# tomas-gr/RawNanoporeSignalCompression

Hardware: AMD Instinct MI355X
Metric: MSamples/s encode+decode (1/2/4/8 GPU) at fixed ratio; % HBM roofline (higher is better)
Workload: dtype int16; 1 GPU; configs[1]: 100000 reads x 100000 int16 samples per GPU (1 chunk each), C5 encode+decode; reads_per_gpu=100000, samples_per_read=100000, global_reads=100000, parallelism=dp1 (reads round-robin, no data-path collective)

## Files before the change

rawnanoporesignalcompression_amd/csrc/pgn_kernels.hip:

```cpp
#include <hip/hip_runtime.h>
#include <stdio.h>
#include <stdlib.h>
#include <string.h>

#include <algorithm>
#include <condition_variable>
#include <mutex>
#include <vector>

#include "../../include/pgnano_hip.h"
#include "../../include/pgnano_pod5.h"
#include "pgn_c5.h"
#include "pgn_internal.h"
#include "pgn_select.h"
#include "pgn_vbz.h"
#include "pgn_variants.h"
#include "pgn_zdec.h"
#include "pgn_zenc.h"

namespace pgn {

constexpr uint32_t kPassSamples = 262144;
static_assert(PGN_MAX_CHUNK_SAMPLES >= kPassSamples, "chunk limits");
constexpr uint32_t kMaxEncSeq = (uint32_t)z1::kMaxSrc / 4 + 2;
// ... 2140 lines not shown
    case kCodecC4: hipLaunchKernelGGL(enc_chunk_kernel<kCodecC4>, dim3((unsigned)slots), dim3(64), 0, s, a); break;
    case kCodecC1: hipLaunchKernelGGL(enc_chunk_kernel<kCodecC1>, dim3((unsigned)slots), dim3(64), 0, s, a); break;
    case kCodecC2: hipLaunchKernelGGL(enc_chunk_kernel<kCodecC2>, dim3((unsigned)slots), dim3(64), 0, s, a); break;
    case kCodecC3: hipLaunchKernelGGL(enc_chunk_kernel<kCodecC3>, dim3((unsigned)slots), dim3(64), 0, s, a); break;
    case kCodecVbz0: hipLaunchKernelGGL(enc_chunk_kernel<kCodecVbz0>, dim3((unsigned)slots), dim3(64), 0, s, a); break;
    default: return PGN_ERR_INVALID_ARG;
    }
    HIPCHK(hipGetLastError());
    return PGN_OK;
}

static int launch_decode_fused(pgn_ctx* c, int codec, size_t nchunks, const uint8_t* d_in, const uint64_t* d_in_offsets,
                               const uint64_t* d_in_sizes, const DecOut& d_samples, const uint64_t* d_sample_offsets,
                               const uint32_t* d_sample_counts, int32_t* d_status, hipStream_t s)
{
    const size_t slots = nchunks < c->decFusedSlotsMax ? nchunks : c->decFusedSlotsMax;
    int rc = ensure_dec(c, slots, 0);
    if (rc) return rc;
    HIPCHK(hipEventRecord(c->ev[2], s));
    rc = ensure_queues(c, 1, s);
    if (rc) return rc;
    DecArgs a{};
    a.nchunks = nchunks;
    a.in = d_in;
    a.inOffsets = d_in_offsets;
    a.inSizes = d_in_sizes;
    set_out(a, d_samples);
    a.sampleOffsets = d_sample_offsets;
    a.sampleCounts = d_sample_counts;
    a.status = d_status;
    a.slotScratch = c->decScratch;
    a.slotBytes = dec_slot_bytes();
    a.prof = c->prof ? c->prof + kPhases : nullptr;
    a.queue = c->qCur;
    a.capN = kPassSamples;
    a.list = nullptr;
    c->lastUnits = nullptr;
    return launch_dec_chunks(codec, a, slots, s);
}

static int launch_dec_chunks(int codec, const DecArgs& a, size_t slots, hipStream_t s)
{
    switch (codec) {
    case kCodecC5: hipLaunchKernelGGL(dec_chunk_kernel<kCodecC5>, dim3((unsigned)slots), dim3(64), 0, s, a); break;
    case kCodecVbz: hipLaunchKernelGGL(dec_chunk_kernel<kCodecVbz>, dim3((unsigned)slots), dim3(64), 0, s, a); break;
    case kCodecC4: hipLaunchKernelGGL(dec_chunk_kernel<kCodecC4>, dim3((unsigned)slots), dim3(64), 0, s, a); break;
    case kCodecC1: hipLaunchKernelGGL(dec_chunk_kernel<kCodecC1>, dim3((unsigned)slots), dim3(64), 0, s, a); break;
    case kCodecC2: hipLaunchKernelGGL(dec_chunk_kernel<kCodecC2>, dim3((unsigned)slots), dim3(64), 0, s, a); break;
    case kCodecC3: hipLaunchKernelGGL(dec_chunk_kernel<kCodecC3>, dim3((unsigned)slots), dim3(64), 0, s, a); break;
    case kCodecVbz0: hipLaunchKernelGGL(dec_chunk_kernel<kCodecVbz0>, dim3((unsigned)slots), dim3(64), 0, s, a); break;
    default: return PGN_ERR_INVALID_ARG;
    }
    HIPCHK(hipGetLastError());
    return PGN_OK;
}

static int launch_encode_impl(pgn_ctx* c, int codec, size_t nchunks, const int16_t* d_samples, const uint64_t* d_sample_offsets,
                         const uint32_t* d_sample_counts, uint8_t* d_out, const uint64_t* d_out_offsets,
                         const uint64_t* d_out_caps, uint64_t* d_out_sizes, int32_t* d_status, uint64_t* d_stats,
                         void* stream)
{
    HIPCHK(hipSetDevice(c->device));
    hipStream_t s = stream ? (hipStream_t)stream : c->stream;
    const bool staged = c->encStaged || (!c->encForced && nchunks <= c->encStagedBelow);
    if (!staged || (codec != kCodecC5 && codec != kCodecVbz))
        return launch_encode_fused(c, codec, nchunks, d_samples, d_sample_offsets, d_sample_counts, d_out, d_out_offsets,
                                   d_out_caps, d_out_sizes, d_status, d_stats, s);
    const size_t G = nchunks < c->subBatch ? nchunks : c->subBatch;
    const size_t passes = (nchunks + G - 1) / G;
    const uint32_t nu = codec == kCodecVbz ? 1u : (uint32_t)kStreams;
    const size_t slots = nu * G < c->encSlotsMax ? nu * G : c->encSlotsMax;
    const size_t nbuf = passes > 1 ? 2 : 1;
    int rc = ensure_enc(c, slots, nbuf * G);
    if (rc) return rc;
    HIPCHK(hipEventRecord(c->ev[0], s));
    rc = ensure_queues(c, passes, s);
    if (rc) return rc;
    const hipStream_t sideS = passes > 1 ? c->side : s;
    if (passes > 1) {
        HIPCHK(hipEventRecord(c->evFork, s));
        HIPCHK(hipStreamWaitEvent(c->side, c->evFork, 0));
    }
    const size_t bufBytes = G * (kChunkStreamBytes + kChunkFrameBytes + 2 * 4 * kStreams);
    EncArgs a;
    a.nchunks = nchunks;
    a.samples = d_samples;
    a.sampleOffsets = d_sample_offsets;
    a.sampleCounts = d_sample_counts;
    a.out = d_out;
    a.outOffsets = d_out_offsets;
    a.outCaps = d_out_caps;
    a.outSizes = d_out_sizes;
    a.status = d_status;
    a.stats = d_stats;
    a.slotScratch = c->encScratch;
    a.slotBytes = enc_slot_bytes();
    a.epochs = c->epochs;
    a.prof = c->prof;
    a.G = G;
    a.nu = nu;
    a.capN = kPassSamples;
    a.list = nullptr;
    a.lookback = nullptr;
    a.epoch = 0;
    if (passes == 1 && G <= kSplitWgMaxChunks && codec != kCodecVbz) {
        rc = take_lookback(c, s, a.lookback, a.epoch);
        if (rc) return rc;
    }
    for (size_t p = 0; p < passes; p++) {
        const int b = (int)(p & 1);
        uint8_t* buf = c->encChunks + (size_t)b * bufBytes;
        a.streams = buf;
        a.frames = buf + G * kChunkStreamBytes;
        a.sizes = (uint32_t*)(a.frames + G * kChunkFrameBytes);
        a.fsizes = a.sizes + G * kStreams;
        a.base = p * G;
        a.queue = c->qCur + p;
        if (p >= 2) HIPCHK(hipStreamWaitEvent(c->side, c->evFree[b], 0));
        if (codec == kCodecVbz) hipLaunchKernelGGL(vbz_split_kernel, dim3((unsigned)G), dim3(64), 0, sideS, a);
        else if (a.lookback)
            hipLaunchKernelGGL(enc_split_lb_kernel, dim3((unsigned)(G * kSplitRanges)), dim3(64), 0, sideS, a);
        else hipLaunchKernelGGL(enc_split_kernel, dim3((unsigned)G), dim3(64), 0, sideS, a);
        if (passes > 1) {
            HIPCHK(hipEventRecord(c->evStage[b], c->side));
            HIPCHK(hipStreamWaitEvent(s, c->evStage[b], 0));
        }
        const bool coop = G <= kSplitWgMaxChunks && (size_t)nu * G <= slots;
        if (coop)
            hipLaunchKernelGGL(enc_zstd_coop_kernel, dim3((unsigned)(nu * G)), dim3(64 * kCoopEncWaves), 0, s, a);
        else hipLaunchKernelGGL(enc_zstd_kernel, dim3((unsigned)slots), dim3(64), 0, s, a);
        if (codec == kCodecVbz) hipLaunchKernelGGL(vbz_assemble_kernel, dim3((unsigned)G), dim3(64), 0, s, a);
        else if (!(coop && a.lookback)) hipLaunchKernelGGL(enc_assemble_kernel, dim3((unsigned)G), dim3(64), 0, s, a);
        if (passes > 1) HIPCHK(hipEventRecord(c->evFree[b], s));
    }
    HIPCHK(hipGetLastError());
    return PGN_OK;
}

#define PGN_LAUNCH_MERGE_PA(T)                                                                                           \
    do {                                                                                                                 \
        if (codec == kCodecVbz) hipLaunchKernelGGL(vbz_merge_pa_kernel<T>, dim3((unsigned)G), dim3(64), 0, ms, a);       \
        else if (a.lookback)                                                                                             \
            hipLaunchKernelGGL(dec_merge_lb_pa_kernel<T>, dim3((unsigned)(G * kMergeRanges)), dim3(64), 0, ms, a);       \
        else hipLaunchKernelGGL(dec_merge_pa_kernel<T>, dim3((unsigned)G), dim3(64), 0, ms, a);                          \
    } while (0)
static void launch_merge(int codec, const DecArgs& a, size_t G, hipStream_t ms)
{
    if (a.outType == PGN_OUT_F32) PGN_LAUNCH_MERGE_PA(float);
    else if (a.outType == PGN_OUT_F16) PGN_LAUNCH_MERGE_PA(_Float16);
    else if (codec == kCodecVbz) hipLaunchKernelGGL(vbz_merge_kernel, dim3((unsigned)G), dim3(64), 0, ms, a);
    else if (a.lookback)
        hipLaunchKernelGGL(dec_merge_lb_kernel, dim3((unsigned)(G * kMergeRanges)), dim3(64), 0, ms, a);
    else hipLaunchKernelGGL(dec_merge_kernel, dim3((unsigned)G), dim3(64), 0, ms, a);
}

static int launch_decode_impl(pgn_ctx* c, int codec, size_t nchunks, const uint8_t* d_in, const uint64_t* d_in_offsets,
                         const uint64_t* d_in_sizes, const DecOut& d_samples, const uint64_t* d_sample_offsets,
                         const uint32_t* d_sample_counts, int32_t* d_status, void* stream, uint32_t capCall)
{
    HIPCHK(hipSetDevice(c->device));
    hipStream_t s = stream ? (hipStream_t)stream : c->stream;
    if (!c->decStaged || (codec != kCodecC5 && codec != kCodecVbz))
        return launch_decode_fused(c, codec, nchunks, d_in, d_in_offsets, d_in_sizes, d_samples, d_sample_offsets,
                                   d_sample_counts, d_status, s);
    bool defer = codec == kCodecC5 && nchunks >= c->deferMin;
    const size_t stride = chunk_inter_bytes(capCall);
    size_t G = nchunks < c->subBatch ? nchunks : c->subBatch;
// ... 1186 lines not shown
```

rawnanoporesignalcompression_amd/csrc/pgn_zenc.h:

```cpp
#pragma once
#ifndef PGN_AB_SKIP
#define PGN_AB_SKIP 0
#endif
#include "pgn_c5.h"
#include "pgn_wave.h"
#include "zstd1_model.h"

namespace pgn {

constexpr int kWinWords = 392;
constexpr int kFiltSlots = 512;

struct WCTable {
    uint32_t tableLog;
    uint16_t stateTable[64];
    uint32_t deltaNbBits[16];
    int32_t deltaFindState[16];
};

struct alignas(16) EncLds {
    union {
        struct {
            uint64_t filt[kFiltSlots];
            uint32_t vh0[64], vh1[64], vpk[64];
            uint32_t vd0[64], vd1[64];
        };
        struct {
            uint32_t hist2[2][256];
            union {
            uint32_t hist2x[1 + 2 * 256];
            struct {
            uint8_t nbBits[256];
            uint16_t val[256];
            union {
                struct {
                    z1::HufNode nodes[2 * 256 + 4];
                    union {
                        uint32_t count[256];
                        struct {
                            uint16_t tanc[256];
                            uint16_t tdep[256];
                        };
                    };
                    uint32_t rankLast[16];
                    uint32_t vpr[16];
                };
                struct {
                    uint8_t weights[256];
                    uint8_t hdr[256];
                    WCTable fct;
                    uint8_t fscratch[64];
                    uint32_t wcount[16];
                    int16_t wnorm[16];
                    uint32_t wcumul[16];
                };
                struct {
                    uint32_t win[kWinWords];
                    uint32_t cw[256];
                };
            };
            };
            };
        };
        struct {
            z1::FseCTable sct[3];
            uint8_t stsym[512];
            uint32_t scount[3][64];
            int16_t snorm[64];
            uint32_t scumul[64];
            uint8_t snc[128];
            uint32_t sv[3][64];
            uint8_t sc[3][64];
        };
    };
    uint32_t u[8];
};
__device__ __forceinline__ uint32_t seg_count(const EncLds& L, int k, int s)
{
    return (L.hist2[k >> 1][s] >> (16 * (k & 1))) & 0xFFFFu;
}

static_assert(sizeof(EncLds) <= kCodecLdsBytes, "encoder LDS exceeds the codec LDS");
static_assert(__builtin_offsetof(EncLds, hdr) % 4 == 0, "table description words");
#define sEnc (*reinterpret_cast<EncLds*>(sCodecLds))

struct EncScratch {
    uint32_t* ht;
    z1::Seq* seqs;
    uint8_t* codes;
    uint8_t* lit;
    uint8_t* seqSection;
    z1::SeqWork* seqWork;
    uint32_t maxSeq;
    uint32_t* huf;
    struct CoopEncCmd __attribute__((address_space(3)))* coop;
};

__device__ inline uint32_t wave_match_count(const uint8_t* src, uint32_t a, uint32_t b, uint32_t end)
{
    const uint32_t o = 4u * (uint32_t)lane_id();
    uint32_t n = 0;
    while (a + n < end) {
        const uint32_t len = end - (a + n);
        const uint32_t nv = len > o ? (len - o < 4u ? len - o : 4u) : 0u;
        const int32_t so = (int32_t)len - 4 < (int32_t)o ? (int32_t)len - 4 : (int32_t)o;
        const uint32_t wa = ld32u(src + (int64_t)(a + n) + so), wb = ld32u(src + (int64_t)(b + n) + so);
        const uint32_t sh = 8u * (uint32_t)((int32_t)o - so);
        uint32_t x = nv ? ((wa ^ wb) >> sh) : 0u;
        x &= nv >= 4u ? 0xFFFFFFFFu : ((1u << (8u * nv)) - 1u);
        const uint32_t mism = x ? o + ((uint32_t)__builtin_ctz(x) >> 3) : 0xFFFFFFFFu;
        const uint64_t mm = ballot(mism != 0xFFFFFFFFu);
        if (mm) return n + readlane_u32(mism, __builtin_ctzll(mm));
        if (len <= 256u) return len + n;
        n += 256;
    }
    return n;
}

constexpr uint32_t kTagShift = 27;
constexpr uint32_t kTagEpochs = 1u << (32 - kTagShift);
constexpr uint32_t kMaxIdxBits = 26;
constexpr size_t kMaxFrameBytes = ((size_t)1 << kMaxIdxBits) - 2;
__host__ __device__ inline uint32_t ht_idx_bits(uint32_t frameN)
{
    if (frameN + 2 < (1u << 17)) return 17u;
    if (frameN + 2 < (1u << 20)) return 20u;
    uint32_t b = 21;
    while (b < kMaxIdxBits && frameN + 2 >= (1u << b)) b++;
    return b;
}
__device__ inline uint32_t ht_fp(uint32_t bytes, uint32_t idxBits)
{
    return ((bytes * 0x9E3779B1u) >> (32u - (kTagShift - idxBits))) << idxBits;
}
__device__ inline uint32_t ht_entry(uint32_t tag, uint32_t idx, uint32_t bytes, uint32_t idxBits)
{
    return (tag << kTagShift) | ht_fp(bytes, idxBits) | idx;
}
__device__ __forceinline__ void ht_next_epoch(uint32_t* ht, uint32_t& st, uint32_t n)
{
    uint32_t ep = (st & 0xFFu) + 1u, dirty = st >> 8;
    if (ep >= kTagEpochs) {
        for (uint32_t i = (uint32_t)lane_id(); i < ((1u << dirty) >> 2); i += 64) gst<uint4>(ht + 4 * i, make_uint4(0, 0, 0, 0));
        ep = 1;
        dirty = 0;
        wave_sync();
    }
    if (n >= 7) {
        const uint32_t hl = z1::level1_params(n).hashLog;
        dirty = hl > dirty ? hl : dirty;
    }
    st = ep | (dirty << 8);
}

__device__ __forceinline__ uint32_t hash_g(const uint8_t* p, unsigned hlog, unsigned mls)
// ... 812 lines not shown
    }
    for (uint32_t b = 0; b <= maxNbBits; b++) {
        uint32_t base = L.vpr[b];
#pragma unroll
        for (int j = 0; j < 4; j++) {
            const uint64_t m = ballot(nbS[j] == b);
            if (nbS[j] == b) val[j] = base + mbcnt(m);
            base += (uint32_t)__builtin_popcountll(m);
        }
    }
#pragma unroll
    for (int j = 0; j < 4; j++) {
        const uint32_t s = (uint32_t)lane + 64u * (uint32_t)j;
        if (s <= maxSym) L.val[s] = (uint16_t)val[j];
    }
    lds_sync();
    return maxNbBits;
}

__device__ __forceinline__ void fse_build_ctable_small(WCTable& ct, const int16_t* norm, unsigned maxSymbolValue,
                                                       unsigned tableLog, uint8_t* tableSymbol, uint32_t* cumul)
{
    (void)cumul;
    const uint32_t lane = (uint32_t)lane_id();
    const uint32_t tableSize = 1u << tableLog;
    const uint32_t tableMask = tableSize - 1;
    const uint32_t step = (tableSize >> 1) + (tableSize >> 3) + 3;
    ct.tableLog = tableLog;
    const int nv = (lane <= maxSymbolValue) ? (int)norm[lane] : 0;
    const bool low = nv == -1;
    const uint32_t cnt = low ? 1u : (nv > 0 ? (uint32_t)nv : 0u);
    const uint32_t excl = wave_incl_sum(cnt) - cnt;
    const uint64_t lowMask = ballot(low);
    if (low) tableSymbol[tableSize - 1 - mbcnt(lowMask)] = (uint8_t)lane;
    const uint32_t highThreshold = tableSize - 1 - (uint32_t)__builtin_popcountll(lowMask);
    const uint32_t ncnt = low ? 0u : cnt;
    const uint32_t nincl = wave_incl_sum(ncnt);
    const uint32_t pos = (lane * step) & tableMask;
    const bool valid = lane < tableSize && pos <= highThreshold;
    const uint32_t k = mbcnt(ballot(valid));
    uint32_t sym = 0;
    for (uint32_t q = 0; q <= maxSymbolValue; q++) sym += readlane_u32(nincl, (int)q) <= k ? 1u : 0u;
    if (valid) tableSymbol[pos] = (uint8_t)sym;
    lds_sync();
    const bool isEntry = lane < tableSize;
    const uint32_t sy = isEntry ? tableSymbol[lane] : 0xFFu;
    uint32_t rank = 0;
    for (uint32_t q = 0; q <= maxSymbolValue; q++) {
        const uint64_t m = ballot(sy == q);
        if (sy == q) rank = mbcnt(m);
    }
    const uint32_t cs = (uint32_t)__shfl((int)excl, (int)(sy & 63u), 64);
    if (isEntry) ct.stateTable[cs + rank] = (uint16_t)(tableSize + lane);
    if (lane <= maxSymbolValue) {
        if (nv == 0) {
            ct.deltaNbBits[lane] = ((tableLog + 1) << 16) - (1u << tableLog);
            ct.deltaFindState[lane] = 0;
        } else if (nv == -1 || nv == 1) {
            ct.deltaNbBits[lane] = (tableLog << 16) - (1u << tableLog);
            ct.deltaFindState[lane] = (int32_t)excl - 1;
        } else {
            const uint32_t maxBitsOut = tableLog - z1::highbit32((uint32_t)(nv - 1));
            const uint32_t minStatePlus = (uint32_t)nv << maxBitsOut;
            ct.deltaNbBits[lane] = (maxBitsOut << 16) - minStatePlus;
            ct.deltaFindState[lane] = (int32_t)excl - nv;
        }
    }
    lds_sync();
}

__device__ __forceinline__ void wfse_init(uint32_t& st, const WCTable& ct, unsigned symbol)
{
    const uint32_t nbBitsOut = (ct.deltaNbBits[symbol] + (1u << 15)) >> 16;
    const uint32_t v = (nbBitsOut << 16) - ct.deltaNbBits[symbol];
    st = ct.stateTable[(v >> nbBitsOut) + ct.deltaFindState[symbol]];
}
__device__ __forceinline__ void wfse_encode(z1::BitW& bw, uint32_t& st, const WCTable& ct, unsigned symbol)
{
    const uint32_t nbBitsOut = (st + ct.deltaNbBits[symbol]) >> 16;
    z1::bw_add(bw, st, nbBitsOut);
    st = ct.stateTable[(st >> nbBitsOut) + ct.deltaFindState[symbol]];
}

__device__ __noinline__ uint32_t huf_write_ctable_wave(uint32_t maxSym, uint32_t huffLog, PhaseProf& P)
{
    EncLds& L = sEnc;
    const int lane = lane_id();
    maxSym = uni(maxSym);
    huffLog = uni(huffLog);
    const uint32_t wtSize = maxSym;
    uint32_t w[4];
#pragma unroll
    for (int j = 0; j < 4; j++) {
        const uint32_t s = (uint32_t)lane + 64u * (uint32_t)j;
        w[j] = 0xFFu;
        if (s < wtSize) {
            const uint32_t nb = L.nbBits[s];
            w[j] = nb ? huffLog + 1 - nb : 0u;
            L.weights[s] = (uint8_t)w[j];
        }
    }
    for (uint32_t v = 0; v <= z1::kHufTableLogMax; v++) {
        uint32_t c = 0;
#pragma unroll
        for (int j = 0; j < 4; j++) c += (uint32_t)__builtin_popcountll(ballot(w[j] == v));
        if (lane == 0) L.wcount[v] = c;
    }
    lds_sync();
    uint32_t hSize = 0;
    if (wtSize > 1) {
        unsigned maxW = z1::kHufTableLogMax;
        while (!L.wcount[maxW]) maxW--;
        uint32_t maxCount = 0;
        for (unsigned v = 0; v <= maxW; v++) maxCount = L.wcount[v] > maxCount ? L.wcount[v] : maxCount;
        if (maxCount == wtSize) {
            hSize = 1;
        } else if (maxCount > 1) {
            const unsigned tableLog = z1::fse_optimal_table_log(6, wtSize, maxW, 2);
            if (z1::fse_normalize(L.wnorm, tableLog, L.wcount, wtSize, maxW, false)) {
                lds_sync();
                const size_t nh = z1::fse_write_ncount(L.hdr + 1, L.wnorm, maxW, tableLog);
                if (nh && wtSize > 2) {
                    fse_build_ctable_small(L.fct, L.wnorm, maxW, tableLog, L.fscratch, L.wcumul);
                    const uint32_t vST = ((uint32_t)lane < (1u << tableLog)) ? (uint32_t)L.fct.stateTable[lane] : 0u;
                    const uint32_t vDN = ((uint32_t)lane <= maxW) ? L.fct.deltaNbBits[lane] : 0u;
                    const uint32_t vDF = ((uint32_t)lane <= maxW) ? (uint32_t)L.fct.deltaFindState[lane] : 0u;
                    const uint32_t W4 = reinterpret_cast<const uint32_t*>(L.weights)[lane];
                    auto wsym = [&](uint32_t i) -> uint32_t {
                        return (readlane_u32(W4, (int)(i >> 2)) >> (8u * (i & 3u))) & 0xFFu;
                    };
                    auto init = [&](uint32_t sym) -> uint32_t {
                        const uint32_t dn = readlane_u32(vDN, (int)sym), df = readlane_u32(vDF, (int)sym);
                        const uint32_t nbo = (dn + (1u << 15)) >> 16;
                        const uint32_t v = (nbo << 16) - dn;
                        return readlane_u32(vST, (int)((v >> nbo) + df));
                    };
                    const uint32_t n = wtSize, nEm = n - 2;
                    uint32_t dnR[4], dfR[4], rec[4];
#pragma unroll
                    for (int r = 0; r < 4; r++) {
                        const uint32_t k = (uint32_t)lane + 64u * (uint32_t)r;
                        const uint32_t sy = k < nEm ? (uint32_t)L.weights[n - 3 - k] : 0u;
                        dnR[r] = L.fct.deltaNbBits[sy];
                        dfR[r] = (uint32_t)L.fct.deltaFindState[sy];
                        rec[r] = 0;
                    }
                    uint32_t stX = init(wsym(n - 1)), stY = init(wsym(n - 2));
                    auto enc = [&](uint32_t& st, uint32_t& rc, uint32_t dv, uint32_t fv, uint32_t k) {
                        const uint32_t dn = readlane_u32(dv, (int)(k & 63u)), df = readlane_u32(fv, (int)(k & 63u));
                        const uint32_t nbo = (st + dn) >> 16;
                        asm volatile("v_writelane_b32 %0, %1, m0" : "+v"(rc) : "s"(st | (nbo << 16)), "{m0}"(k & 63u));
                        st = readlane_u32(vST, (int)((st >> nbo) + df));
                    };
#pragma unroll
                    for (uint32_t r = 0; r < 4; r++) {
                        const uint32_t kEnd = nEm < 64u * r + 64u ? nEm : 64u * r + 64u;
                        for (uint32_t k = 64u * r; k < kEnd; k += 2) {
                            enc(stX, rec[r], dnR[r], dfR[r], k);
                            if (k + 1 < kEnd) enc(stY, rec[r], dnR[r], dfR[r], k + 1);
                        }
                    }
                    const uint32_t fA = ((n & 1u) ? stY : stX) | (tableLog << 16), fB = ((n & 1u) ? stX : stY) | (tableLog << 16);
                    uint32_t pos[4], tot = 0;
#pragma unroll
                    for (int r = 0; r < 4; r++) {
                        const uint32_t k = (uint32_t)lane + 64u * (uint32_t)r;
                        if (k == nEm) rec[r] = fA;
                        if (k == nEm + 1) rec[r] = fB;
                        if (k == nEm + 2) rec[r] = 1u | (1u << 16);
                        const uint32_t nb = k < nEm + 3 ? rec[r] >> 16 : 0u;
                        const uint32_t incl = wave_incl_sum(nb);
                        pos[r] = tot + incl - nb;
                        tot += readlane_u32(incl, 63);
                    }
                    const uint32_t bytes = (tot + 7) >> 3;
                    uint8_t* op = L.hdr + 1 + nh;
                    for (uint32_t b = (uint32_t)lane; b < bytes; b += 64) op[b] = 0;
                    lds_sync();
                    lds_u32* hw = (lds_u32*)(uint32_t*)L.hdr;
                    const uint32_t B0 = 8u * (1u + (uint32_t)nh);
#pragma unroll
                    for (int r = 0; r < 4; r++) {
                        const uint32_t k = (uint32_t)lane + 64u * (uint32_t)r;
                        if (k < nEm + 3) {
                            const uint32_t nb = rec[r] >> 16, v = rec[r] & ((1u << nb) - 1u);
                            const uint32_t P = B0 + pos[r], w = P >> 5, sh = P & 31u;
                            __hip_atomic_fetch_or(&hw[w], v << sh, __ATOMIC_RELAXED, __HIP_MEMORY_SCOPE_WAVEFRONT);
                            if (sh + nb > 32u)
                                __hip_atomic_fetch_or(&hw[w + 1], v >> (32u - sh), __ATOMIC_RELAXED, __HIP_MEMORY_SCOPE_WAVEFRONT);
                        }
                    }
                    hSize = (uint32_t)(nh + bytes);
                }
            }
        }
    }
    lds_sync();
    if (hSize > 1 && hSize < maxSym / 2) {
        if (lane == 0) L.hdr[0] = (uint8_t)hSize;
        lds_sync();
        return hSize + 1;
    }
    if (maxSym > 128) return 0;
    if (lane == 0) L.hdr[0] = (uint8_t)(128 + (maxSym - 1));
    if ((uint32_t)lane < (maxSym + 1) / 2) {
        const uint32_t a = L.weights[2 * lane], b = (2u * (uint32_t)lane + 1u < maxSym) ? L.weights[2 * lane + 1] : 0u;
        L.hdr[1 + lane] = (uint8_t)((a << 4) + b);
    }
    lds_sync();
    return (maxSym + 1) / 2 + 1;
}

__device__ __forceinline__ void fse_build_ctable_lds(z1::FseCTable& ct, const int16_t* norm, unsigned maxSymbolValue,
                                                     unsigned tableLog, uint8_t* tableSymbol, uint32_t* cumul)
{
    const uint32_t tableSize = 1u << tableLog;
    const uint32_t tableMask = tableSize - 1;
    const uint32_t step = (tableSize >> 1) + (tableSize >> 3) + 3;
    uint32_t highThreshold = tableSize - 1;
    ct.tableLog = tableLog;
    cumul[0] = 0;
    for (unsigned u = 1; u <= maxSymbolValue + 1; u++) {
        if (norm[u - 1] == -1) {
            cumul[u] = cumul[u - 1] + 1;
            tableSymbol[highThreshold--] = (uint8_t)(u - 1);
        } else {
            cumul[u] = cumul[u - 1] + (uint32_t)norm[u - 1];
        }
    }
    cumul[maxSymbolValue + 1] = tableSize + 1;
    uint32_t position = 0;
    for (unsigned symbol = 0; symbol <= maxSymbolValue; symbol++) {
        const int freq = norm[symbol];
        for (int k = 0; k < freq; k++) {
            tableSymbol[position] = (uint8_t)symbol;
            position = (position + step) & tableMask;
            while (position > highThreshold) position = (position + step) & tableMask;
        }
    }
    lds_sync();
    for (uint32_t u = 0; u < tableSize; u++) {
        const uint8_t sy = tableSymbol[u];
        const uint32_t cs = cumul[sy];
        ct.stateTable[cs] = (uint16_t)(tableSize + u);
        cumul[sy] = cs + 1;
    }
    unsigned total = 0;
    for (unsigned sy = 0; sy <= maxSymbolValue; sy++) {
        const int nv = norm[sy];
        if (nv == 0) {
            ct.deltaNbBits[sy] = ((tableLog + 1) << 16) - (1u << tableLog);
            ct.deltaFindState[sy] = 0;
        } else if (nv == -1 || nv == 1) {
            ct.deltaNbBits[sy] = (tableLog << 16) - (1u << tableLog);
            ct.deltaFindState[sy] = (int32_t)total - 1;
            total++;
        } else {
            const uint32_t maxBitsOut = tableLog - z1::highbit32((uint32_t)(nv - 1));
            const uint32_t minStatePlus = (uint32_t)nv << maxBitsOut;
            ct.deltaNbBits[sy] = (maxBitsOut << 16) - minStatePlus;
            ct.deltaFindState[sy] = (int32_t)total - nv;
            total += (unsigned)nv;
        }
    }
    lds_sync();
}

struct GBitW {
    uint8_t* p;
    uint64_t acc;
    uint32_t n;
};
__device__ __forceinline__ void gbw_add(GBitW& b, uint32_t v, uint32_t nb)
{
    b.acc |= (uint64_t)(v & (uint32_t)((1ull << nb) - 1ull)) << b.n;
    b.n += nb;
    if (b.n >= 32) {
        if (lane_id() == 0) gst<uint32_t>(b.p, (uint32_t)b.acc);
        b.p += 4;
        b.acc >>= 32;
        b.n -= 32;
    }
}
__device__ __forceinline__ size_t gbw_close(GBitW& b, const uint8_t* start)
{
    gbw_add(b, 1, 1);
    const uint32_t nbytes = (b.n + 7) >> 3;
    if (lane_id() == 0)
        for (uint32_t i = 0; i < nbytes; i++) gst<uint8_t>(b.p + i, (uint8_t)(b.acc >> (8 * i)));
    return (size_t)(b.p + nbytes - start);
}
__device__ __forceinline__ void sfse_init(uint32_t& st, const z1::FseCTable& ct, unsigned symbol)
{
    const uint32_t nbBitsOut = (ct.deltaNbBits[symbol] + (1u << 15)) >> 16;
    const uint32_t v = (nbBitsOut << 16) - ct.deltaNbBits[symbol];
    st = ct.stateTable[(v >> nbBitsOut) + ct.deltaFindState[symbol]];
}
__device__ __forceinline__ void sfse_encode(GBitW& bw, uint32_t& st, const z1::FseCTable& ct, unsigned symbol)
{
    const uint32_t nbBitsOut = (st + ct.deltaNbBits[symbol]) >> 16;
    gbw_add(bw, st, nbBitsOut);
    st = ct.stateTable[(st >> nbBitsOut) + ct.deltaFindState[symbol]];
}

__device__ z1::FseCTable gSeqDefCT[3];
static_assert(sizeof(z1::FseCTable) % 4 == 0, "word copy");
__global__ __launch_bounds__(64) void seq_default_ctables_kernel()
{
    EncLds& L = sEnc;
    const int lane = lane_id();
#pragma unroll 1
    for (int k = 0; k < 3; k++) {
        const unsigned dmax = k == 0 ? z1::kMaxLL : (k == 1 ? z1::kDefaultMaxOff : z1::kMaxML);
        const unsigned lg = k == 0 ? z1::kLLDefaultNormLog : (k == 1 ? z1::kOFDefaultNormLog : z1::kMLDefaultNormLog);
        if ((unsigned)lane <= dmax)
            L.snorm[lane] = k == 0 ? z1::ll_default_norm(lane) : (k == 1 ? z1::of_default_norm(lane) : z1::ml_default_norm(lane));
        lds_sync();
        fse_build_ctable_lds(L.sct[k], L.snorm, dmax, lg, L.stsym, L.scumul);
        const uint32_t* w = (const uint32_t*)&L.sct[k];
        for (uint32_t u = (uint32_t)lane; u < sizeof(z1::FseCTable) / 4; u += 64) ((uint32_t*)&gSeqDefCT[k])[u] = w[u];
        lds_sync();
    }
}

__device__ __noinline__ size_t seq_section_wave(EncScratch S, uint32_t nbSeq)
{
    EncLds& L = sEnc;
    const uint32_t lane = (uint32_t)lane_id();
    nbSeq = uni(nbSeq);
    S.seqs = uni(S.seqs);
    S.codes = uni(S.codes);
    S.seqSection = uni(S.seqSection);
    S.maxSeq = uni(S.maxSeq);
    uint8_t* const dst = S.seqSection;
    uint8_t* llC = S.codes;
    uint8_t* ofC = S.codes + S.maxSeq;
    uint8_t* mlC = S.codes + 2 * S.maxSeq;
    const uint32_t* sq = (const uint32_t*)S.seqs;
    uint32_t hl;
    if (nbSeq < 128) {
        if (lane == 0) gst<uint8_t>(dst, (uint8_t)nbSeq);
        hl = 1;
    } else if (nbSeq < 0x7F00) {
        if (lane == 0) { gst<uint8_t>(dst, (uint8_t)((nbSeq >> 8) + 0x80)); gst<uint8_t>(dst + 1, (uint8_t)nbSeq); }
        hl = 2;
    } else {
        if (lane == 0) { gst<uint8_t>(dst, 0xFF); gst<uint8_t>(dst + 1, (uint8_t)(nbSeq - 0x7F00)); gst<uint8_t>(dst + 2, (uint8_t)((nbSeq - 0x7F00) >> 8)); }
        hl = 3;
    }
    if (nbSeq == 0) return hl;
    uint8_t* const seqHead = dst + hl;
    uint8_t* op = seqHead + 1;
    for (int k = 0; k < 3; k++) L.scount[k][lane] = 0;
    lds_sync();
    for (uint32_t i = lane; i < nbSeq; i += 64) {
        const uint32_t litLength = gld<uint32_t>(sq + 3 * i), offset = gld<uint32_t>(sq + 3 * i + 1),
                       mlBase = gld<uint32_t>(sq + 3 * i + 2);
        const uint32_t lc = z1::ll_code(litLength), oc = z1::highbit32(offset), mc = z1::ml_code(mlBase);
        gst<uint8_t>(llC + i, (uint8_t)lc);
        gst<uint8_t>(ofC + i, (uint8_t)oc);
        gst<uint8_t>(mlC + i, (uint8_t)mc);
        atomicAdd(&L.scount[0][lc], 1u);
        atomicAdd(&L.scount[1][oc], 1u);
        atomicAdd(&L.scount[2][mc], 1u);
    }
    lds_sync();
    const uint32_t last = nbSeq - 1;
    const uint32_t lastLL = gld<uint32_t>(sq + 3 * last), lastOff = gld<uint32_t>(sq + 3 * last + 1),
                   lastML = gld<uint32_t>(sq + 3 * last + 2);
    const uint32_t lastCode[3] = {z1::ll_code(lastLL), z1::highbit32(lastOff), z1::ml_code(lastML)};
    uint8_t* lastNCount = nullptr;
    uint32_t types[3];
    const unsigned maxes[3] = {z1::kMaxLL, z1::kMaxOff, z1::kMaxML};
    const unsigned fseLogs[3] = {z1::kLLFSELog, z1::kOffFSELog, z1::kMLFSELog};
    const unsigned normLogs[3] = {z1::kLLDefaultNormLog, z1::kOFDefaultNormLog, z1::kMLDefaultNormLog};
#pragma unroll
    for (int k = 0; k < 3; k++) {
        const uint32_t cnt = (lane <= maxes[k]) ? L.scount[k][lane] : 0u;
        const uint64_t nz = ballot(cnt != 0);
        const unsigned mx = 63u - (unsigned)__builtin_clzll(nz);
        const uint32_t mostFrequent = wave_max(cnt);
        const bool defaultAllowed = (k == 1) ? (mx <= z1::kDefaultMaxOff) : true;
        const unsigned type = z1::select_encoding_type(mostFrequent, nbSeq, normLogs[k], defaultAllowed);
        types[k] = type;
        z1::FseCTable& ct = L.sct[k];
        if (type == z1::kSetRle) {
            ct.tableLog = 0;
            ct.stateTable[0] = 0;
            ct.stateTable[1] = 0;
            ct.deltaNbBits[mx] = 0;
            ct.deltaFindState[mx] = 0;
            if (lane == 0) gst<uint8_t>(op, (uint8_t)lastCode[k]);
            op += 1;
        } else if (type == z1::kSetBasic) {
            const uint32_t* w = (const uint32_t*)&gSeqDefCT[k];
            for (uint32_t u = lane; u < sizeof(z1::FseCTable) / 4; u += 64) ((uint32_t*)&ct)[u] = gld<uint32_t>(w + u);
        } else {
            size_t nbSeq_1 = nbSeq;
            const unsigned tableLog = z1::fse_optimal_table_log(fseLogs[k], nbSeq, mx, 2);
            if (L.scount[k][lastCode[k]] > 1) {
                L.scount[k][lastCode[k]] -= 1;
                nbSeq_1--;
            }
            lds_sync();
            if (!z1::fse_normalize(L.snorm, tableLog, L.scount[k], nbSeq_1, mx, nbSeq_1 >= 2048)) return (size_t)-2;
            lds_sync();
            const size_t nc = z1::fse_write_ncount(L.snc, L.snorm, mx, tableLog);
            if (nc == 0) return (size_t)-2;
            lds_sync();
            for (uint32_t i = lane; i < nc; i += 64) gst<uint8_t>(op + i, L.snc[i]);
            fse_build_ctable_lds(ct, L.snorm, mx, tableLog, L.stsym, L.scumul);
            lastNCount = op;
            op += nc;
        }
        lds_sync();
    }
    if (lane == 0) gst<uint8_t>(seqHead, (uint8_t)((types[0] << 6) + (types[1] << 4) + (types[2] << 2)));
    GBitW bw{op, 0, 0};
    uint32_t sLL, sOF, sML;
    sfse_init(sML, L.sct[2], lastCode[2]);
    sfse_init(sOF, L.sct[1], lastCode[1]);
// ... 150 lines not shown
#endif
    if (largest == n) {
        size_t fl = z1::raw_lit_header_size(n);
        if (lane == 0) {
            z1::write_rawrle_lit_header(dst, n, z1::kSetRle);
            dst[fl] = lit[0];
        }
        return ret(fl + 1, false);
    }
    if (largest <= (n >> 7) + 4) { size_t r = write_raw_literals_wave(dst, lit, n); P.mark(7); return ret(r, false); }
    uint32_t oldNb[4] = {0, 0, 0, 0};
    bool repeat = false;
    if (prevCheck) {
        bool bad = false;
#pragma unroll
        for (int q = 0; q < 4; q++) {
            oldNb[q] = gld<uint32_t>(prevCw + lane + 64 * q) >> 16;
            bad |= c[q] != 0 && oldNb[q] == 0;
        }
        repeat = !ballot(bad);
    }
    bool useOld = repeat && n <= 1024;
    uint32_t hSize = 0;
    if (!useOld) {
    unsigned huffLog = z1::huf_optimal_table_log(z1::kHufTableLogDefault, n, maxSym);
    for (int i = lane; i < 2 * 256 + 4; i += 64) {
        L.nodes[i].count = 0; L.nodes[i].parent = 0; L.nodes[i].byte = 0; L.nodes[i].nbBits = 0;
    }
    wave_sync();
    {
        uint32_t a[4];
#pragma unroll
        for (int q = 0; q < 4; q++) {
            const uint32_t sy = (uint32_t)lane + 64u * (uint32_t)q;
            a[q] = (sy <= maxSym) ? ~((c[q] << 8) | (255u - sy)) : 0xFFFFFFFFu;
        }
#pragma unroll
        for (uint32_t k = 2; k <= 256; k <<= 1) {
#pragma unroll
            for (uint32_t j = k >> 1; j > 0; j >>= 1) {
                if (j >= 64) {
                    const uint32_t qj = j >> 6;
#pragma unroll
                    for (uint32_t q = 0; q < 4; q++) {
                        if (q & qj) continue;
                        const uint32_t q2 = q | qj;
                        const uint32_t mn = a[q] < a[q2] ? a[q] : a[q2], mx = a[q] < a[q2] ? a[q2] : a[q];
                        const bool asc = ((64u * q) & k) == 0;
                        a[q] = asc ? mn : mx;
                        a[q2] = asc ? mx : mn;
                    }
                } else {
#pragma unroll
                    for (uint32_t q = 0; q < 4; q++) {
                        const uint32_t b = (uint32_t)__shfl_xor((int)a[q], (int)j, 64);
                        const uint32_t mn = a[q] < b ? a[q] : b, mx = a[q] < b ? b : a[q];
                        const uint32_t e = (uint32_t)lane + 64u * q;
                        const bool lower = (e & j) == 0, asc = (e & k) == 0;
                        a[q] = (lower == asc) ? mn : mx;
                    }
                }
            }
        }
#pragma unroll
        for (int q = 0; q < 4; q++) {
            const uint32_t r = (uint32_t)lane + 64u * (uint32_t)q;
            if (r <= maxSym) {
                const uint32_t key = ~a[q];
                L.nodes[1 + r].count = key >> 8;
                L.nodes[1 + r].byte = (uint8_t)(255u - (key & 0xFFu));
            }
        }
    }
    wave_sync();
    P.mark(4);
    uint32_t nnz = 0;
#pragma unroll
    for (int q = 0; q < 4; q++) nnz += (uint32_t)__builtin_popcountll(ballot(c[q] != 0));
    const uint32_t hl = huf_tree_wave(maxSym, huffLog, nnz, P);
    P.mark(14);
#if PGN_AB_SKIP == 5
    { size_t r = write_raw_literals_wave(dst, lit, n); return ret(r + 0 * hl, false); }
#endif
    if (!repeat) {
        uint32_t b4[4] = {0, 0, 0, 0};
#pragma unroll
        for (int q = 0; q < 4; q++) {
            const int s = lane + 64 * q;
            const uint32_t nbq = ((uint32_t)s <= maxSym) ? (uint32_t)L.nbBits[s] : 0u;
#pragma unroll
            for (int k = 0; k < 4; k++) b4[k] += seg_count(L, k, s) * nbq;
        }
        uint32_t cs = single ? 0u : 6u;
#pragma unroll
        for (int k = 0; k < 4; k++)
            if (k == 0 || !single) cs += (wave_sum(b4[k]) + 8) >> 3;
        if (cs >= n - minGain) { size_t r = write_raw_literals_wave(dst, lit, n); P.mark(7); return ret(r, false); }
        if (lhSize + cs >= rawAt) { P.mark(7); return ret(lhSize + cs, false); }
    }
    hSize = huf_write_ctable_wave(maxSym, hl, P);
    P.count(5);
    P.count(6, maxSym);
    P.mark(5);
    if (hSize == 0) { size_t r = write_raw_literals_wave(dst, lit, n); P.mark(7); return ret(r, false); }
    if (repeat) {
        uint32_t eo = 0, en = 0;
#pragma unroll
        for (int q = 0; q < 4; q++) {
            const int s = lane + 64 * q;
            eo += c[q] * oldNb[q];
            en += c[q] * (((uint32_t)s <= maxSym) ? (uint32_t)L.nbBits[s] : 0u);
        }
        const uint32_t oldSize = wave_sum(eo) >> 3, newSize = wave_sum(en) >> 3;
        useOld = oldSize <= hSize + newSize || hSize + 12 >= n;
    }
    if (!useOld && hSize + 12 >= n) { size_t r = write_raw_literals_wave(dst, lit, n); P.mark(7); return ret(r, false); }
    }
    if (useOld) hSize = 0;
    uint32_t bytes[4] = {0, 0, 0, 0}, bits[4] = {0, 0, 0, 0};
    {
        uint32_t b4[4] = {0, 0, 0, 0};
#pragma unroll
        for (int q = 0; q < 4; q++) {
            int s = lane + 64 * q;
            uint32_t cwq;
            if (useOld) cwq = gld<uint32_t>(prevCw + s);
            else cwq = ((uint32_t)s <= maxSym) ? ((uint32_t)L.val[s] | ((uint32_t)L.nbBits[s] << 16)) : 0u;
            L.cw[s] = cwq;
            const uint32_t nbq = cwq >> 16;
#pragma unroll
            for (int k = 0; k < 4; k++) b4[k] += seg_count(L, k, s) * nbq;
        }
#pragma unroll
        for (int k = 0; k < 4; k++) {
            bits[k] = wave_sum(b4[k]);
            bytes[k] = (bits[k] + 8) >> 3;
        }
    }
    uint32_t cStreams = single ? bytes[0] : 6 + bytes[0] + bytes[1] + bytes[2] + bytes[3];
    uint32_t total = hSize + cStreams;
    if (total >= n - 1 || total >= n - minGain) { size_t r = write_raw_literals_wave(dst, lit, n); P.mark(7); return ret(r, false); }
    if (lhSize + total >= rawAt) { P.mark(7); return ret(lhSize + total, false); }
    if (!useOld && saveNew) {
#pragma unroll
        for (int q = 0; q < 4; q++) gst<uint32_t>(nextCw + lane + 64 * q, L.cw[lane + 64 * q]);
    }
    if (lane == 0) {
        z1::write_huf_lit_header(dst, lhSize, n, total, single, useOld ? z1::kSetRepeat : z1::kSetCompressed);
        if (!single) {
            z1::wr16(dst + lhSize + hSize, bytes[0]);
            z1::wr16(dst + lhSize + hSize + 2, bytes[1]);
            z1::wr16(dst + lhSize + hSize + 4, bytes[2]);
        }
    }
    for (uint32_t i = (uint32_t)lane; i < hSize; i += 64) gst<uint8_t>(dst + lhSize + i, L.hdr[i]);
    wave_sync();
    uint8_t* op = dst + lhSize + hSize + (single ? 0 : 6);
    if (COOP && !single) {
        if (lane == 0) {
            coop->op = 2;
            coop->lit = lit;
            coop->n = n;
            coop->segSize = segSize;
            uint8_t* o = op;
            for (int k = 0; k < 4; k++) {
                coop->out[k] = o;
                coop->bits[k] = bits[k];
                o += bytes[k];
            }
        }
        __syncthreads();
        huf_encode_segment_wave(op, lit, segSize, bits[0], (lds_u32*)sEnc.win);
        __syncthreads();
    } else {
        for (int k = 0; k < nseg; k++) {
            uint32_t a = segSize * (uint32_t)k;
            uint32_t e = (k == nseg - 1) ? n : a + segSize;
#if PGN_AB_SKIP != 4
            huf_encode_segment_wave(op, lit + a, e - a, bits[k], (lds_u32*)sEnc.win);
#endif
            P.count(7, (e - a + 1023) / 1024);
            op += bytes[k];
        }
// ... 143 lines not shown
```

Baseline: 224,500 MSamples/s.

## Add single-batch sequence encoder, early-exit Huffman weight table, LDS-based FSE chain

```diff
diff --git a/rawnanoporesignalcompression_amd/csrc/pgn_kernels.hip b/rawnanoporesignalcompression_amd/csrc/pgn_kernels.hip
--- a/rawnanoporesignalcompression_amd/csrc/pgn_kernels.hip
+++ b/rawnanoporesignalcompression_amd/csrc/pgn_kernels.hip
@@ -2246,7 +2246,7 @@
         HIPCHK(hipStreamWaitEvent(c->side, c->evFork, 0));
     }
     const size_t bufBytes = G * (kChunkStreamBytes + kChunkFrameBytes + 2 * 4 * kStreams);
-    EncArgs a;
+    EncArgs a{};
     a.nchunks = nchunks;
     a.samples = d_samples;
     a.sampleOffsets = d_sample_offsets;
diff --git a/rawnanoporesignalcompression_amd/csrc/pgn_zenc.h b/rawnanoporesignalcompression_amd/csrc/pgn_zenc.h
--- a/rawnanoporesignalcompression_amd/csrc/pgn_zenc.h
+++ b/rawnanoporesignalcompression_amd/csrc/pgn_zenc.h
@@ -53,6 +53,8 @@
                     uint32_t wcount[16];
                     int16_t wnorm[16];
                     uint32_t wcumul[16];
+                    uint2 wpair[256];
+                    uint32_t wrec[256];
                 };
                 struct {
                     uint32_t win[kWinWords];
@@ -64,13 +66,18 @@
         };
         struct {
             z1::FseCTable sct[3];
-            uint8_t stsym[512];
             uint32_t scount[3][64];
-            int16_t snorm[64];
-            uint32_t scumul[64];
-            uint8_t snc[128];
-            uint32_t sv[3][64];
-            uint8_t sc[3][64];
+            union {
+                struct {
+                    uint8_t stsym[512];
+                    int16_t snorm[64];
+                    uint32_t scumul[64];
+                    uint8_t snc[128];
+                    uint32_t sv[3][64];
+                    uint8_t sc[3][64];
+                };
+                uint2 spair[3][64];
+            };
         };
     };
     uint32_t u[8];
@@ -1049,12 +1056,13 @@
     st = ct.stateTable[(st >> nbBitsOut) + ct.deltaFindState[symbol]];
 }
 
-__device__ __noinline__ uint32_t huf_write_ctable_wave(uint32_t maxSym, uint32_t huffLog, PhaseProf& P)
+__device__ __noinline__ uint32_t huf_write_ctable_wave(uint32_t maxSym, uint32_t huffLog, uint32_t rawFrom, PhaseProf& P)
 {
     EncLds& L = sEnc;
     const int lane = lane_id();
     maxSym = uni(maxSym);
     huffLog = uni(huffLog);
+    rawFrom = uni(rawFrom);
     const uint32_t wtSize = maxSym;
     uint32_t w[4];
 #pragma unroll
@@ -1087,45 +1095,59 @@
             if (z1::fse_normalize(L.wnorm, tableLog, L.wcount, wtSize, maxW, false)) {
                 lds_sync();
                 const size_t nh = z1::fse_write_ncount(L.hdr + 1, L.wnorm, maxW, tableLog);
-                if (nh && wtSize > 2) {
+                bool chain = nh && wtSize > 2;
+                if (chain) {
+                    const uint32_t wl0 = L.weights[wtSize - 1], wl1 = L.weights[wtSize - 2];
+                    uint32_t mb = 0;
+                    if ((uint32_t)lane <= maxW) {
+                        const uint32_t c = L.wcount[lane] - (wl0 == (uint32_t)lane) - (wl1 == (uint32_t)lane);
+                        const int nv = L.wnorm[lane];
+                        mb = c * (nv <= 1 ? tableLog : tableLog - z1::highbit32((uint32_t)(nv - 1)) - 1u);
+                    }
+                    const uint32_t hLow = (uint32_t)nh + ((wave_sum(mb) + 2u * tableLog + 1u + 7u) >> 3);
+                    if (hLow >= maxSym / 2) {
+                        hSize = hLow;
+                        chain = false;
+                    } else if (hLow + 1 >= rawFrom && (maxSym > 128 || (maxSym + 1) / 2 + 1 >= rawFrom)) {
+                        return 0;
+                    }
+                }
+                if (chain) {
                     fse_build_ctable_small(L.fct, L.wnorm, maxW, tableLog, L.fscratch, L.wcumul);
-                    const uint32_t vST = ((uint32_t)lane < (1u << tableLog)) ? (uint32_t)L.fct.stateTable[lane] : 0u;
-                    const uint32_t vDN = ((uint32_t)lane <= maxW) ? L.fct.deltaNbBits[lane] : 0u;
-                    const uint32_t vDF = ((uint32_t)lane <= maxW) ? (uint32_t)L.fct.deltaFindState[lane] : 0u;
-                    const uint32_t W4 = reinterpret_cast<const uint32_t*>(L.weights)[lane];
-                    auto wsym = [&](uint32_t i) -> uint32_t {
-                        return (readlane_u32(W4, (int)(i >> 2)) >> (8u * (i & 3u))) & 0xFFu;
-                    };
-                    auto init = [&](uint32_t sym) -> uint32_t {
-                        const uint32_t dn = readlane_u32(vDN, (int)sym), df = readlane_u32(vDF, (int)sym);
-                        const uint32_t nbo = (dn + (1u << 15)) >> 16;
-                        const uint32_t v = (nbo << 16) - dn;
-                        return readlane_u32(vST, (int)((v >> nbo) + df));
-                    };
                     const uint32_t n = wtSize, nEm = n - 2;
-                    uint32_t dnR[4], dfR[4], rec[4];
 #pragma unroll
                     for (int r = 0; r < 4; r++) {
                         const uint32_t k = (uint32_t)lane + 64u * (uint32_t)r;
-                        const uint32_t sy = k < nEm ? (uint32_t)L.weights[n - 3 - k] : 0u;
-                        dnR[r] = L.fct.deltaNbBits[sy];
-                        dfR[r] = (uint32_t)L.fct.deltaFindState[sy];
-                        rec[r] = 0;
+                        if (k < nEm) {
+                            const uint32_t sy = L.weights[n - 3 - k];
+                            L.wpair[k] = make_uint2(L.fct.deltaNbBits[sy], 2u * (uint32_t)L.fct.deltaFindState[sy]);
+                        }
                     }
-                    uint32_t stX = init(wsym(n - 1)), stY = init(wsym(n - 2));
-                    auto enc = [&](uint32_t& st, uint32_t& rc, uint32_t dv, uint32_t fv, uint32_t k) {
-                        const uint32_t dn = readlane_u32(dv, (int)(k & 63u)), df = readlane_u32(fv, (int)(k & 63u));
-                        const uint32_t nbo = (st + dn) >> 16;
-                        asm volatile("v_writelane_b32 %0, %1, m0" : "+v"(rc) : "s"(st | (nbo << 16)), "{m0}"(k & 63u));
-                        st = readlane_u32(vST, (int)((st >> nbo) + df));
-                    };
-#pragma unroll
-                    for (uint32_t r = 0; r < 4; r++) {
-                        const uint32_t kEnd = nEm < 64u * r + 64u ? nEm : 64u * r + 64u;
-                        for (uint32_t k = 64u * r; k < kEnd; k += 2) {
-                            enc(stX, rec[r], dnR[r], dfR[r], k);
-                            if (k + 1 < kEnd) enc(stY, rec[r], dnR[r], dfR[r], k + 1);
-                        }
+                    lds_sync();
+                    uint32_t st = 0;
+                    if (lane < 2) {
+                        const uint32_t sym = L.weights[n - 1 - (uint32_t)lane];
+                        const uint32_t dn0 = L.fct.deltaNbBits[sym], nbo0 = (dn0 + (1u << 15)) >> 16;
+                        st = L.fct.stateTable[(((nbo0 << 16) - dn0) >> nbo0) + (uint32_t)L.fct.deltaFindState[sym]];
+                        auto enc = [&](uint32_t k) {
+                            const uint2 d = L.wpair[k];
+                            const uint32_t nbo = (st + d.x) >> 16;
+                            L.wrec[k] = st | (nbo << 16);
+                            st = *(const uint16_t*)((const uint8_t*)L.fct.stateTable + (2u * (st >> nbo) + d.y));
+                        };
+                        const uint32_t nPair = uni(nEm >> 1);
+                        uint32_t k = (uint32_t)lane;
+#pragma unroll 4
+                        for (uint32_t i = 0; i < nPair; i++, k += 2) enc(k);
+                        if (k < nEm) enc(k);
+                    }
+                    lds_sync();
+                    const uint32_t stX = readlane_u32(st, 0), stY = readlane_u32(st, 1);
+                    uint32_t rec[4];
+#pragma unroll
+                    for (int r = 0; r < 4; r++) {
+                        const uint32_t k = (uint32_t)lane + 64u * (uint32_t)r;
+                        rec[r] = k < nEm ? L.wrec[k] : 0u;
                     }
                     const uint32_t fA = ((n & 1u) ? stY : stX) | (tableLog << 16), fB = ((n & 1u) ? stX : stY) | (tableLog << 16);
                     uint32_t pos[4], tot = 0;
@@ -1290,6 +1312,125 @@
     }
 }
 
+constexpr size_t kSeqNotOneBatch = (size_t)-3;
+__device__ __noinline__ size_t seq_section_one_batch_wave(const uint32_t* sq, uint32_t nbSeq, uint8_t* dst)
+{
+    EncLds& L = sEnc;
+    const uint32_t lane = (uint32_t)lane_id();
+    const uint32_t last = nbSeq - 1;
+    const bool act = lane < nbSeq;
+    uint32_t val[3] = {0, 0, 0}, code[3] = {0, 0, 0};
+    if (act) {
+        const uint32_t t = last - lane;
+        val[0] = gld<uint32_t>(sq + 3 * t);
+        val[1] = gld<uint32_t>(sq + 3 * t + 1);
+        val[2] = gld<uint32_t>(sq + 3 * t + 2);
+        code[0] = z1::ll_code(val[0]);
+        code[1] = z1::highbit32(val[1]);
+        code[2] = z1::ml_code(val[2]);
+    }
+#pragma unroll
+    for (int k = 0; k < 3; k++) L.scount[k][lane] = 0;
+    lds_sync();
+    if (act) {
+#pragma unroll
+        for (int k = 0; k < 3; k++) atomicAdd(&L.scount[k][code[k]], 1u);
+    }
+    lds_sync();
+    const unsigned normLogs[3] = {z1::kLLDefaultNormLog, z1::kOFDefaultNormLog, z1::kMLDefaultNormLog};
+    uint32_t types[3];
+#pragma unroll
+    for (int k = 0; k < 3; k++) {
+        const uint32_t mostFrequent = wave_max(act ? L.scount[k][code[k]] : 0u);
+        const uint32_t mx = wave_max(code[k]);
+        types[k] = z1::select_encoding_type(mostFrequent, nbSeq, normLogs[k], k == 1 ? mx <= z1::kDefaultMaxOff : true);
+        if (types[k] == z1::kSetCompressed) return kSeqNotOneBatch;
+    }
+    lds_sync();
+    lds_u32* win = (lds_u32*)&L.scount[0][0];
+#pragma unroll
+    for (int k = 0; k < 3; k++) win[lane + 64 * k] = 0;
+    uint8_t* op = dst + 2;
+    uint32_t tlog[3];
+#pragma unroll
+    for (int k = 0; k < 3; k++) {
+        uint2 d = make_uint2(0u, 0u);
+        if (types[k] == z1::kSetRle) {
+            if (lane == 0) {
+                gst<uint8_t>(op, (uint8_t)code[k]);
+                L.sct[k].stateTable[0] = 0;
+            }
+            op += 1;
+            tlog[k] = 0;
+        } else {
+            if (lane < 32) ((uint32_t*)L.sct[k].stateTable)[lane] = gld<uint32_t>((const uint32_t*)gSeqDefCT[k].stateTable + lane);
+            if (act) d = make_uint2(gld<uint32_t>(&gSeqDefCT[k].deltaNbBits[code[k]]), gld<uint32_t>(&gSeqDefCT[k].deltaFindState[code[k]]));
+            tlog[k] = normLogs[k];
+        }
+        if (act) L.spair[k][lane] = d;
+    }
+    if (lane == 0) {
+        gst<uint8_t>(dst, (uint8_t)nbSeq);
+        gst<uint8_t>(dst + 1, (uint8_t)((types[0] << 6) + (types[1] << 4) + (types[2] << 2)));
+    }
+    lds_sync();
+    uint32_t st = 0;
+    if (lane < 3) {
+        const uint16_t* tbl = L.sct[lane].stateTable;
+        const uint2 d0 = L.spair[lane][0];
+        const uint32_t nbo0 = (d0.x + (1u << 15)) >> 16;
+        st = tbl[(int32_t)(((nbo0 << 16) - d0.x) >> nbo0) + (int32_t)d0.y];
+        for (uint32_t j = 1; j <= last; j++) {
+            const uint2 d = L.spair[lane][j];
+            const uint32_t nbo = (st + d.x) >> 16;
+            L.spair[lane][j].x = st | (nbo << 16);
+            st = tbl[(int32_t)(st >> nbo) + (int32_t)d.y];
+        }
+    }
+    lds_sync();
+    uint32_t fv[6] = {0, 0, 0, val[0], val[2], val[1]}, fn[6] = {0, 0, 0, 0, 0, 0};
+    if (act) {
+        if (lane > 0) {
+            const uint32_t rOF = L.spair[1][lane].x, rML = L.spair[2][lane].x, rLL = L.spair[0][lane].x;
+            fv[0] = rOF & 0xFFFFu; fn[0] = rOF >> 16;
+            fv[1] = rML & 0xFFFFu; fn[1] = rML >> 16;
+            fv[2] = rLL & 0xFFFFu; fn[2] = rLL >> 16;
+        }
+        fn[3] = z1::ll_bits(code[0]);
+        fn[4] = z1::ml_bits(code[2]);
+        fn[5] = code[1];
+    }
+    const uint32_t mine = fn[0] + fn[1] + fn[2] + fn[3] + fn[4] + fn[5];
+    const uint32_t incl = wave_incl_sum(mine);
+    uint32_t pos = incl - mine;
+    auto put = [&](uint32_t at, uint32_t v, uint32_t nb) {
+        if (nb) {
+            v &= (uint32_t)((1ull << nb) - 1ull);
+            const uint32_t w = at >> 5, sh = at & 31u;
+            __hip_atomic_fetch_or(&win[w], v << sh, __ATOMIC_RELAXED, __HIP_MEMORY_SCOPE_WAVEFRONT);
+            if (sh + nb > 32u) __hip_atomic_fetch_or(&win[w + 1], v >> (32u - sh), __ATOMIC_RELAXED, __HIP_MEMORY_SCOPE_WAVEFRONT);
+        }
+    };
+#pragma unroll
+    for (int f = 0; f < 6; f++) {
+        put(pos, fv[f], fn[f]);
+        pos += fn[f];
+    }
+    uint32_t tot = readlane_u32(incl, 63);
+    const uint32_t sLL = readlane_u32(st, 0), sOF = readlane_u32(st, 1), sML = readlane_u32(st, 2);
+    if (lane == 0) {
+        put(tot, sML, tlog[2]);
+        put(tot + tlog[2], sOF, tlog[1]);
+        put(tot + tlog[2] + tlog[1], sLL, tlog[0]);
+        put(tot + tlog[2] + tlog[1] + tlog[0], 1u, 1u);
+    }
+    tot += tlog[2] + tlog[1] + tlog[0] + 1u;
+    lds_sync();
+    const uint32_t bytes = (tot + 7) >> 3;
+    for (uint32_t b = lane; b < bytes; b += 64) gst<uint8_t>(op + b, (uint8_t)(win[b >> 2] >> (8u * (b & 3u))));
+    return (size_t)(op + bytes - dst);
+}
+
 __device__ __noinline__ size_t seq_section_wave(EncScratch S, uint32_t nbSeq)
 {
     EncLds& L = sEnc;
@@ -1304,6 +1445,10 @@
     uint8_t* ofC = S.codes + S.maxSeq;
     uint8_t* mlC = S.codes + 2 * S.maxSeq;
     const uint32_t* sq = (const uint32_t*)S.seqs;
+    if (nbSeq >= 1 && nbSeq <= 64) {
+        const size_t r = seq_section_one_batch_wave(sq, nbSeq, dst);
+        if (r != kSeqNotOneBatch) return r;
+    }
     uint32_t hl;
     if (nbSeq < 128) {
         if (lane == 0) gst<uint8_t>(dst, (uint8_t)nbSeq);
@@ -1620,6 +1765,7 @@
 #if PGN_AB_SKIP == 5
     { size_t r = write_raw_literals_wave(dst, lit, n); return ret(r + 0 * hl, false); }
 #endif
+    uint32_t rawFrom = ~0u;
     if (!repeat) {
         uint32_t b4[4] = {0, 0, 0, 0};
 #pragma unroll
@@ -1635,8 +1781,9 @@
             if (k == 0 || !single) cs += (wave_sum(b4[k]) + 8) >> 3;
         if (cs >= n - minGain) { size_t r = write_raw_literals_wave(dst, lit, n); P.mark(7); return ret(r, false); }
         if (lhSize + cs >= rawAt) { P.mark(7); return ret(lhSize + cs, false); }
-    }
-    hSize = huf_write_ctable_wave(maxSym, hl, P);
+        rawFrom = n - minGain - cs < n - 12 ? n - minGain - cs : n - 12;
+    }
+    hSize = huf_write_ctable_wave(maxSym, hl, rawFrom, P);
     P.count(5);
     P.count(6, maxSym);
     P.mark(5);
```

Result: faster. 228,700 MSamples/s, median of 6 (+1.9%).
